# guomc9/CudaRayTracing

Hardware: AMD Instinct MI355X
Metric: Mrays/sec (higher is better)
Workload: dtype f32

## Files before the change

cudaraytracing_amd/csrc/crt_internal.h:

```cpp
#ifndef CRT_INTERNAL_H
#define CRT_INTERNAL_H
#include <cstdlib>
#include "crt_mega3.h"

#include <cstddef>
#include <string>
#include <vector>

extern "C" void crt_set_last_error_(const char* msg);

namespace crtk {

struct HipFail {
    hipError_t e;
    const char* what;
};
#define HIP_CHECK(call)                                          \
    do {                                                         \
        hipError_t e_ = (call);                                  \
        if (e_ != hipSuccess) throw HipFail{e_, #call};          \
    } while (0)

inline int fail(int status, const std::string& msg)
{
    crt_set_last_error_(msg.c_str());
    return status;
}
inline int fail_hip(const HipFail& f) { return fail(CRT_ERR_HIP, std::string(f.what) + ": " + hipGetErrorString(f.e)); }
template <class Body> int hip_guard(Body body)
{
    try { return body(); } catch (const HipFail& f) { return fail_hip(f); }
}

template <typename T> struct DevBuf {
    T* p = nullptr;
    size_t n = 0;
    void alloc(size_t count)
    {
        release();
        if (count == 0) count = 1;
        HIP_CHECK(hipMalloc((void**)&p, count * sizeof(T)));
        n = count;
        debug_fill();
    }
    void debug_fill()
    {
        static const char* e = std::getenv("CRT_DEBUG_FILL");
        if (!e || !*e) return;
        if (e[0] == 's') { HIP_CHECK(hipDeviceSynchronize()); return; }
        if (e[0] == 'u' && !uncached) return;
        if (e[0] == 'c' && uncached) return;
        const char* v = (e[0] == 'u' || e[0] == 'c') ? e + 1 : e;
        HIP_CHECK(hipMemset(p, std::atoi(v) & 0xff, n * sizeof(T)));
    }
    void ensure(size_t count)
    {
        if (n < count) alloc(count);
    }
    void ensure_uncached(size_t count)
    {
        if (n >= count && uncached) return;
        release();
        if (count == 0) count = 1;
        HIP_CHECK(hipExtMallocWithFlags((void**)&p, count * sizeof(T), hipDeviceMallocUncached));
        n = count;
        uncached = true;
        debug_fill();
    }
    bool uncached = false;
    template <typename Row> T* upload(const std::vector<Row>& v)
    {
        static_assert(sizeof(Row) == sizeof(T) && alignof(T) % alignof(Row) == 0, "upload is a byte copy");
        alloc(v.size());
        if (!v.empty()) HIP_CHECK(hipMemcpy(p, v.data(), v.size() * sizeof(T), hipMemcpyHostToDevice));
        return p;
    }
    T* upload(const T* h, size_t count)
    {
        if (!h) return nullptr;
        alloc(count);
        HIP_CHECK(hipMemcpy(p, h, count * sizeof(T), hipMemcpyHostToDevice));
        return p;
    }
    void download(T* h, size_t count) const
    {
        if (h) HIP_CHECK(hipMemcpy(h, p, count * sizeof(T), hipMemcpyDeviceToHost));
    }
    void release()
    {
        if (p) { (void)hipFree(p); p = nullptr; n = 0; uncached = false; }
    }
    ~DevBuf() { release(); }
};

const int kMaxBatch = 64;

}

#include "crt_stages.h"

namespace crtk {

#define REFILL_MIN 32
#define LEAF_MIN 24
#define SLOT_SHARDS 64
#define SLOT_STRIDE 32
// ... 84 lines not shown
```

cudaraytracing_amd/csrc/crt_mega3.h:

```cpp
#ifndef CRT_MEGA3_H
#define CRT_MEGA3_H
#include "crt_path.h"
#include "crt_item_order.h"

namespace crtk {

struct MParams {
    LParams P;
    DevScene sc;
    unsigned long long* counters;
    int2* spill;
    uint32_t spill_stride;
    int32_t stack_cap;
    int32_t logic_min, leaf_min;
};

#define POOL_LV 4

#define PH3_INNER 0
#define PH3_LEAF 1
#define PH3_LA 2
#define PH3_LB 3
#define PH3_LC 4
#define PH3_N 5
// ... 32 lines not shown
    int node[POOL3_P];
    stk_t stk[LV][POOL3_P];
    uint32_t D[POOL3_P];
    uint8_t ring[PH3_N + 1][POOL3_QCAP];
    uint32_t waitq;
    __device__ __forceinline__ uint8_t* rq(const int p) { return ring[p]; }
};
typedef Pool3LdsT<false> Pool3Lds;
static_assert(sizeof(Pool3LdsT<true>) == sizeof(Pool3Lds), "16-bit stack entries: twice the levels in the same bytes");
static_assert(sizeof(Pool3Lds) * 4 * CRT_WAVES <= 160 * 1024, "the pool does not fit CRT_WAVES waves per SIMD into 160 KiB of LDS");

#ifndef LEAFQ_CAP
#define LEAFQ_CAP 256
#endif
static_assert((LEAFQ_CAP & (LEAFQ_CAP - 1)) == 0 && LEAFQ_CAP >= 128, "leaf queue: a power of two, room for half a batch of inner steps");
constexpr int LEAFQ_FIRST = 48;
static_assert(LEAFQ_FIRST >= 1 && LEAFQ_FIRST + 64 + 4 <= LEAFQ_CAP, "leaf queue: LEAFQ_FIRST - 1 entries + a reference-arithmetic batch + one lane's four entries must fit LEAFQ_CAP");
constexpr int VISIT2_MIN = 44;
constexpr int CHAIN_MIN = 44;
#define RD_PEND_SHIFT 8
#define RD_PEND_MASK 0x3ff00u
#define RD_FIN 0x8000000u
#define LEAF_REC_MAX 0x7fffffu
template <bool R16_, bool RING_>
struct Pool4LdsT {
    static constexpr bool R16 = R16_;
    static constexpr bool DEC = true;
    static constexpr int P = RING_ ? 148 : 152;
    static constexpr int QCAP = (P + 3) & ~3;
    static constexpr int LV = R16_ ? 6 : 3;
    typedef typename std::conditional<R16_, short, int>::type stk_t;
    float4 A[P];
    float4 B[P];
    unsigned long long best[P];
    stk_t stk[LV][P];
    uint32_t D[P];
    uint32_t leafq[LEAFQ_CAP + 1];
    uint8_t ring[(RING_ ? 5 : 4)][QCAP];
    uint32_t waitq;
    __device__ __forceinline__ uint8_t* rq(const int p) { return ring[p == PH3_INNER ? 0 : p - 1]; }
};
static_assert(sizeof(Pool4LdsT<true, false>) * 4 * CRT_WAVES <= 160 * 1024 && sizeof(Pool4LdsT<true, true>) * 4 * CRT_WAVES <= 160 * 1024 &&
              sizeof(Pool4LdsT<false, false>) * 4 * CRT_WAVES <= 160 * 1024 && sizeof(Pool4LdsT<false, true>) * 4 * CRT_WAVES <= 160 * 1024,
              "the DEC pool does not fit CRT_WAVES waves per SIMD into 160 KiB of LDS");
static_assert(Pool4LdsT<true, false>::P <= 256, "ray ids of a pool must fit a byte");

struct MParams3 {
    MParams M;
    int* spill;
    uint32_t force_exact;
    int32_t dbg_loads, dbg_valu;
};

static_assert(offsetof(MParams3, dbg_loads) == 756 && offsetof(MParams3, dbg_valu) == 760, "tools/bbprof/instrument.py reads the counter buffer's address from these two kernel-argument dwords");


typedef void (*Mega3Kernel)(const MParams3);
struct Mega3Variant {
    uint32_t key;
    Mega3Kernel kern;
    uint32_t pool_p;
    int lds_levels;
};
const Mega3Variant* mega3_variant(int mode, bool stats, bool all, bool query, bool r16, bool ring = false, bool dec = false, bool impl = false);
bool bbprof_launch(Mega3Kernel kern, MParams3 M3, uint32_t blocks, hipStream_t st);
void launch_order_items(bool ring, uint32_t blocks, hipStream_t st, const LParams& P, const OrderClasses& C, uint32_t* list, unsigned int* cnt);

}
#endif
```

cudaraytracing_amd/csrc/crt_mega3_logic.h:

```cpp
#ifndef CRT_MEGA3_LOGIC_H
#define CRT_MEGA3_LOGIC_H
#include "crt_mega3_math.h"
#include "crt_mega3_wave.h"

namespace crtk {

struct NewRay {
    F3 o, d;
    float tl;
    uint32_t kind, flags;
};


template <bool QUERY = false>
__device__ __forceinline__ uint32_t route_done(uint32_t rec_flags)
{
    if (QUERY) return PH3_LC;
    return ((rec_flags >> RR_ROUTE_SHIFT) & 3u) + (uint32_t)PH3_LA;
}
__device__ __forceinline__ uint32_t route_bits(uint32_t nr_flags)
{
    const uint32_t r = (nr_flags & RF_SHADOW) ? ((nr_flags & RF_LAST) ? 1u : 0u) : ((nr_flags & RF_PROBE) ? 0u : 2u);
    return r << RR_ROUTE_SHIFT;
}
// ... 15 lines not shown
    const int ref = (MODE != 1 && finite && !force_exact) ? (IMPL ? sc.root4i : sc.root4) : sc.root3_exact;
    bool answered = false;
    float T = FLT_MAX;
    if (MODE != 1 && nr.kind == RAY_SHADOW) {
        flags |= RF_ANYHIT;
        T = nr.tl;
        answered = !(nr.tl == nr.tl) || nr.tl == -pinf() || (nr.flags & RF_SKIP) != 0;
    }
    if constexpr (LDS::DEC) {
        static_assert(!LDS::DEC || MODE == 2, "decoupled leaves: CRT_TRAVERSAL_EXACT");
        if (ref < 0) flags |= RF_EXACT;
        S.A[id] = make_float4(nr.o.x, nr.o.y, nr.o.z, (flags & RF_ANYHIT) ? T : pinf());
        S.B[id] = make_float4(nr.d.x, nr.d.y, nr.d.z, __int_as_float(ref));
        S.best[id] = (unsigned long long)0x7f7fffffu << 32;
        S.D[id] = flags;
        enters_exact = false;
        if (answered) return route_done<QUERY>(flags);
        enters_exact = (flags & RF_EXACT) != 0;
        return PH3_INNER;
    } else {
    S.A[id] = make_float4(nr.o.x, nr.o.y, nr.o.z, T);
    S.B[id] = make_float4(nr.d.x, nr.d.y, nr.d.z, __int_as_float(-1));
    S.node[id] = ref;
    S.D[id] = flags;
    enters_exact = false;
    if (answered) return route_done<QUERY>(flags);
    enters_exact = MODE != 1 && (flags & RF_EXACT) != 0;
    return ref >= 0 ? PH3_INNER : PH3_LEAF;
    }
}

template <class LDS>
__device__ __forceinline__ void ray_result(LDS& S, const uint32_t id, float4& qa, float4& qb)
{
    qa = S.A[id]; qb = S.B[id];
    if constexpr (LDS::DEC) {
        const unsigned long long b = S.best[id];
        qa.w = __uint_as_float((uint32_t)(b >> 32));
        qb.w = __uint_as_float(~(uint32_t)b);
    }
}
template <bool QUERY>
__device__ __forceinline__ uint32_t route_complete(const uint32_t rec_flags, const bool has_hit)
{
    if (QUERY) return PH3_LC;
    const uint32_t r = (rec_flags >> RR_ROUTE_SHIFT) & 3u;
    return (has_hit ? (r & 1u) : r) + (uint32_t)PH3_LA;
}


#define ST_TL_INF (1u << 12)

__device__ __forceinline__ F3 finish_path_m3(const LParams& P, const Tables<false>& tb, const uint32_t slot, const int deepest, const bool emissive, const F3 ke,
                                            const bool have_ld, const F3 ld)
{
    const Pool& pl = P.pool;
    if (deepest < 0) return f3(0.0f, 0.0f, 0.0f);
    F3 L;
    if (emissive) L = seed_emitter(deepest, ke);
    else if (have_ld) L = seed_direct(ld);
    else {
        const float4 a = gld_rec(&pl.rec_a[(size_t)deepest * pl.n + slot]);
        L = seed_direct(f3(a.x, a.y, a.z));
    }
    for (int v = deepest - 1; v >= 0; v -= CRT_FINISH_PF) {
        float4 a[CRT_FINISH_PF], fm[CRT_FINISH_PF];
        float cs[CRT_FINISH_PF];
#pragma unroll
        for (int j = 0; j < CRT_FINISH_PF; j++) {
            const int vj = v - j > 0 ? v - j : 0;
            a[j] = gld_rec(&pl.rec_a[(size_t)vj * pl.n + slot]);
            cs[j] = gld(&pl.rec_c[(size_t)vj * pl.n + slot]);
        }
#pragma unroll
        for (int j = 0; j < CRT_FINISH_PF; j++) fm[j] = mat_row(tb, TNM_MAT(__float_as_uint(a[j].w)), 0);
#pragma unroll
        for (int j = 0; j < CRT_FINISH_PF; j++) {
            if (v - j >= 0) L = indirect_step(L, f3(fm[j].x, fm[j].y, fm[j].z), cs[j], P.p_rr, f3(a[j].x, a[j].y, a[j].z));
        }
    }
    return L;
}


template <int MODE, bool RING = false>
__device__ __forceinline__ uint32_t logic_A(const LParams& P, const Tables<false>& tb, const uint32_t g, const float4 qa, const float4 qb, NewRay& nr,
                                            PathCounters& cnt, const bool trace_all)
{
    const DevScene& sc = P.sc;
    const Pool& pl = P.pool;
    constexpr bool TRI_CC = MODE != 1;
    const float4 la = gld(&pl.la[g]);
    const uint4 idv = load_path_id<RING, !TRI_CC>(P, g);
    const float4 cc = gld(&pl.cc[g]);
    const uint32_t st = __float_as_uint(la.w);
    const uint32_t stage = (st >> 8) & 15u;
    const uint32_t vtri_old = TRI_CC ? ((st & 0xfffu) == ((uint32_t)ST_HIT << 8) ? 0u : __float_as_uint(cc.w)) : idv.w;
    const float4 vn = gld(&sc.tri_nm[vtri_old]);
    const float res_t = qa.w;
    const int res_tri = __float_as_int(qb.w);
    const float4 gq_hit = gld(&sc.tri_nm[res_tri >= 0 ? res_tri : 0]);
    const uint32_t mat_old = min(TNM_MAT(__float_as_uint(vn.w)), P.n_mats - 1u);
    const uint32_t mat_cur = stage == ST_HIT ? TNM_MAT(__float_as_uint(gq_hit.w)) : mat_old;
    uint32_t tnm_cur = stage == ST_HIT ? __float_as_uint(gq_hit.w) : __float_as_uint(vn.w);
    float4 m0_cur = mat_row(tb, mat_cur, 0);
    const uint32_t n_nee = (uint32_t)(sc.n_lights * P.lsn);
    const uint32_t q_next = stage == ST_SHADOW ? (st >> 16) + 1 : 0u;
    uint4 lg_next = make_uint4(0u, 1u, 0u, 0u);
    if (n_nee > 0) {
        if (sc.n_lights == 1) {
            const crt_u4v_ l0_ = *(const __attribute__((address_space(4))) crt_u4v_*)tb.lights;
            lg_next = make_uint4(l0_.x, l0_.y, l0_.z, l0_.w);
        } else lg_next = gld(&tb.lights[fast_div(q_next < n_nee ? q_next : 0u, P.lsn_div.m, P.lsn_div.sh)]);
    }
    Lane s;
    s.depth = st & 255u; s.q = st >> 16; s.stage = stage;
    s.Ld = f3(la.x, la.y, la.z);
    s.nrm = f3(vn.x, vn.y, vn.z); s.mat = TNM_MAT(__float_as_uint(vn.w));
    s.pixel_index = idv.x; s.k = idv.y; s.item = idv.z;
    s.ro = f3(qa.x, qa.y, qa.z); s.tl = 0.0f;
    s.rd = f3(qb.x, qb.y, qb.z);
    s.pos = s.ro; s.vtri = vtri_old; s.c = f3(0.0f, 0.0f, 0.0f); s.kind = RAY_NONE;
    bool do_enter = false;
    if (stage == ST_SHADOW) {
        const bool blocked = TRI_CC ? shadow_blocked_bit((st & ST_TL_INF) != 0u, res_tri) : shadow_blocked<MODE>(cc.w, res_t, res_tri);
        if (!blocked) s.Ld = add3(s.Ld, f3(cc.x, cc.y, cc.z));
        s.q++;
    } else if (stage == ST_HIT) {
        const F3 pos = add3(s.ro, scalel3(res_t, s.rd));
        do_enter = true;
        if (s.depth > 0) {
            const size_t pr = (size_t)(s.depth - 1) * pl.n + g;
            const F3 pn = s.nrm;
            const float cos_prev = cos_to_next(s.ro, pos, pn);
            gst_rec(&pl.rec_c[pr], cos_prev);
            if (TNM_SPECULAR(__float_as_uint(vn.w))) {
                const float ns = mat_row(tb, s.mat, 0).w;
                const float4 pb = gld_rec(&pl.rec_b[pr]);
                const F3 refd = probe_dir(P.seed, s.pixel_index, s.k, s.depth - 1, ns, f3(pb.x, pb.y, pb.z), pn);
                gst_rec(&pl.rec_b[(size_t)s.depth * pl.n + g], make_float4(s.rd.x, s.rd.y, s.rd.z, 0.0f));
                gst(&pl.vx[g], make_float4(pos.x, pos.y, pos.z, __int_as_float(res_tri)));
                gst(&pl.la[g], make_float4(s.Ld.x, s.Ld.y, s.Ld.z, __uint_as_float(s.depth | ((uint32_t)ST_PROBE << 8) | (s.q << 16))));
                nr.o = s.ro; nr.d = unit3(refd);  nr.tl = 0.0f; nr.kind = RAY_CLOSEST; nr.flags = RF_PROBE;
                return PH3_NONE;
            }
        }
        s.pos = pos; s.vtri = (uint32_t)res_tri;
    } else {
        const float4 vx = gld(&pl.vx[g]);
        s.pos = f3(vx.x, vx.y, vx.z); s.vtri = __float_as_uint(vx.w);
        if (res_tri >= 0) {
            const int hmat = gld(&sc.tri_mat[res_tri]);
            const float4 h1 = mat_row(tb, hmat, 1);
            if (__float_as_uint(h1.w) & 1u) {
                const float4 h2 = mat_row(tb, hmat, 2);
                const size_t pr = (size_t)(s.depth - 1) * pl.n + g;
                const F3 pn = s.nrm;
                const float4 pm0 = mat_row(tb, s.mat, 0), pm1 = mat_row(tb, s.mat, 1);
                const F3 temp = probe_term(pn, f3(pm1.x, pm1.y, pm1.z), f3(h2.x, h2.y, h2.z), s.ro, s.rd, res_t, pm0.w);
                float4 a = gld_rec(&pl.rec_a[pr]);
                a.x = a.x + temp.x; a.y = a.y + temp.y; a.z = a.z + temp.z;
                gst_rec(&pl.rec_a[pr], a);
            }
        }
        const float4 pb = gld_rec(&pl.rec_b[(size_t)s.depth * pl.n + g]);
        s.rd = f3(pb.x, pb.y, pb.z);
        do_enter = true;
    }
    if (do_enter) {
        float4 gq = gq_hit;
        if (stage == ST_PROBE) {
            gq = gld(&sc.tri_nm[s.vtri]);
            m0_cur = mat_row(tb, TNM_MAT(__float_as_uint(gq.w)), 0); tnm_cur = __float_as_uint(gq.w);
        }
        s.nrm = f3(gq.x, gq.y, gq.z);
        s.mat = TNM_MAT(__float_as_uint(gq.w));
        if (TNM_SPECULAR(tnm_cur)) gst_rec(&pl.rec_b[(size_t)s.depth * pl.n + g], make_float4(s.rd.x, s.rd.y, s.rd.z, 0.0f));
        if (!TRI_CC) store_path_tri(P, g, s.vtri);
        if (TNM_EMITTER(tnm_cur)) {
            gst(&pl.la[g], make_float4(TRI_CC ? __uint_as_float(s.vtri) : 0.0f, 0.0f, 0.0f, __uint_as_float(s.depth | ((uint32_t)ST_FIN << 8) | (1u << 16))));
            return PH3_LC;
        }
        s.Ld = f3(0.0f, 0.0f, 0.0f);
        s.q = 0;
        if (n_nee == 0) {
            gst(&pl.la[g], make_float4(0.0f, 0.0f, 0.0f, __uint_as_float(s.depth | ((uint32_t)ST_NEED << 8))));
            if (TRI_CC) gst(&pl.cc[g].w, __uint_as_float(s.vtri));
            nr.o = s.pos;
            return PH3_LB;
        }
    }
    constexpr int LA_LOOP_MIN = 16;
    const float4 m0 = m0_cur;
    bool skip;
    for (bool first = true;; first = false) {
        if (first) setup_shadow_lg(P, s, f3(m0.x, m0.y, m0.z), lg_next);
        else setup_shadow(P, tb, s, f3(m0.x, m0.y, m0.z));
        skip = MODE != 1 && !trace_all && (s.c.x == 0.0f && s.c.y == 0.0f && s.c.z == 0.0f);
        if (!skip) break;
        cnt.untraced++;
        if (__popcll(__builtin_amdgcn_ballot_w64(true)) < LA_LOOP_MIN) break;
        cnt.rays++; cnt.shadow++;
        s.q++;
        if (s.q == n_nee) {
            gst(&pl.la[g], make_float4(s.Ld.x, s.Ld.y, s.Ld.z, __uint_as_float(s.depth | ((uint32_t)ST_NEED << 8))));
            if (TRI_CC) gst(&pl.cc[g].w, __uint_as_float(s.vtri));
            nr.o = s.pos;
            return PH3_LB;
        }
    }
    gst(&pl.la[g], make_float4(s.Ld.x, s.Ld.y, s.Ld.z, __uint_as_float(s.depth | ((uint32_t)ST_SHADOW << 8) | (s.q << 16) | ((TRI_CC && s.tl == pinf()) ? ST_TL_INF : 0u))));
    gst(&pl.cc[g], make_float4(s.c.x, s.c.y, s.c.z, TRI_CC ? __uint_as_float(s.vtri) : s.tl));
    nr.o = s.ro; nr.d = s.rd; nr.tl = s.tl; nr.kind = RAY_SHADOW;
    nr.flags = RF_SHADOW | (s.q + 1 == n_nee ? RF_LAST : 0u) | (skip ? RF_SKIP : 0u);
    return PH3_NONE;
}

template <int MODE, bool RING = false>
__device__ __forceinline__ uint32_t logic_B(const LParams& P, const uint32_t g, const float4 qa, const float4 qb, NewRay& nr)
{
    const Pool& pl = P.pool;
    constexpr bool TRI_CC = MODE != 1;
    const float4 la = gld(&pl.la[g]);
    const uint4 idv = load_path_id<RING, !TRI_CC>(P, g);
    const float4 cc = gld(&pl.cc[g]);
    const uint32_t st = __float_as_uint(la.w);
    const uint32_t stage = (st >> 8) & 15u;
    uint32_t depth = st & 255u;
    F3 Ld = f3(la.x, la.y, la.z);
    if (stage == ST_SHADOW) {
        const bool blocked = TRI_CC ? shadow_blocked_bit((st & ST_TL_INF) != 0u, __float_as_int(qb.w)) : shadow_blocked<MODE>(cc.w, qa.w, __float_as_int(qb.w));
        if (!blocked) Ld = add3(Ld, f3(cc.x, cc.y, cc.z));
    }
    U4 rb;
    if (roulette(P.seed, idv.x, idv.y, depth, P.p_rr, rb)) {
        gst(&pl.la[g], make_float4(Ld.x, Ld.y, Ld.z, __uint_as_float(depth | ((uint32_t)ST_FIN << 8))));
        return PH3_LC;
    }
    const float4 vn = gld(&P.sc.tri_nm[TRI_CC ? __float_as_uint(cc.w) : idv.w]);
    const float4 vx = qa;
    gst_rec(&pl.rec_a[(size_t)depth * pl.n + g], make_float4(Ld.x, Ld.y, Ld.z, vn.w));
    const F3 ndir = bounce_dir(f3(vn.x, vn.y, vn.z), rb);
    depth++;
    gst(&pl.la[g], make_float4(Ld.x, Ld.y, Ld.z, __uint_as_float(depth | ((uint32_t)ST_HIT << 8))));
    nr.o = f3(vx.x, vx.y, vx.z); nr.d = unit3(ndir);  nr.tl = 0.0f; nr.kind = RAY_CLOSEST; nr.flags = 0;
    return PH3_NONE;
}

enum { LC_DEAD = 0, LC_RAY = 1, LC_WAIT = 2 };
template <int MODE, bool RING>
__device__ __forceinline__ int logic_C(const LParams& P, const Tables<false>& tb, const uint32_t g, PathCounters& cnt, NewRay& nr, uint32_t& fin_key)
{
    constexpr bool TRI_CC = MODE != 1;
    const Pool& pl = P.pool;
    const float4 la = gld(&pl.la[g]);
    const uint4 idv = load_path_id<RING, !TRI_CC>(P, g);
    const uint32_t st = __float_as_uint(la.w);
    const uint32_t stage = (st >> 8) & 15u;
    const uint32_t depth = st & 255u;
    constexpr bool ring = RING;
    const bool waiting = ring && stage == ST_WAIT;
    const uint32_t home_ = RING ? blockIdx.x & (P.ring_shards - 1u) : blockIdx.x & (ITEM_SHARDS - 1);
    const uint32_t lo_ = home_ * P.items_per_shard, hi_ = min(lo_ + P.items_per_shard, P.n_items);
    const unsigned long long gmask_ = __ballot(!waiting);
    const int lane_ = threadIdx.x & 63;
    const uint32_t grank_ = (uint32_t)__popcll(gmask_ & ((1ull << lane_) - 1ull));
    unsigned int pre_base_ = 0;
    const bool pre_ok_ = lo_ < P.n_items && gmask_ != 0ull;
    if (pre_ok_ && lane_ == __ffsll((long long)gmask_) - 1) pre_base_ = __hip_atomic_fetch_add((CRT_GAS unsigned int*)(P.item_next + home_ * ITEM_STRIDE), (unsigned int)__popcll(gmask_), __ATOMIC_RELAXED, __HIP_MEMORY_SCOPE_AGENT);
    uint32_t home_word_ = 0;
    if (RING) home_word_ = ring_load(P.ring_state + home_ * ITEM_STRIDE);
    if (stage != ST_NEW && !waiting) {
        int deepest = (int)depth;
        bool emissive = false;
        F3 ke = f3(0.0f, 0.0f, 0.0f);
        if (stage == ST_HIT) deepest = (int)depth - 1;
        else if ((st >> 16) & 1u) {
            emissive = true;
            const float4 m2 = mat_row(tb, TNM_MAT(__float_as_uint(gld(&P.sc.tri_nm[TRI_CC ? __float_as_uint(la.x) : idv.w]).w)), 2);
            ke = f3(m2.x, m2.y, m2.z);
        }
        const F3 L = finish_path_m3(P, tb, g, deepest, emissive, ke, stage == ST_FIN && !emissive, f3(la.x, la.y, la.z));
        if (ring) {
            const uint32_t sh = fast_div(idv.z, P.items_per_shard_div.m, P.items_per_shard_div.sh), c = idv.z - sh * P.items_per_shard;
            const uint32_t s = fast_div(c, P.spsh_div.m, P.spsh_div.sh), rs = s & P.ring_mask;
            Rad3* Lr = P.L + (size_t)rs * P.ring_stride + (size_t)sh * P.spsh + (c - s * P.spsh);
            ring_store12(Lr, L.x, L.y, L.z);
            fin_key = (sh << 16) | rs;
        } else {
            store_radiance(&P.L[idv.z], L.x, L.y, L.z);
        }
    }
    bool first_ = pre_ok_ && !waiting;
    for (;;) {
        uint32_t item = ITEM_NONE;
        if (waiting) item = idv.z;
        else {
            if (first_) {
                const unsigned long long idx_ = (unsigned long long)lo_ + (unsigned int)__builtin_amdgcn_readfirstlane((int)pre_base_) + grank_;
                if (idx_ < hi_) item = (uint32_t)idx_;
                first_ = false;
            }
            if (item == ITEM_NONE) item = RING ? grab_item_ring(P.item_next, P.items_per_shard, P.ring_shards, home_)
                                               : grab_item(P.item_next, P.items_per_shard, P.n_items, blockIdx.x & (ITEM_SHARDS - 1));
            if (item == ITEM_NONE) return LC_DEAD;
            if (P.item_list) {
                const uint32_t sh_ = fast_div(item, P.items_per_shard_div.m, P.items_per_shard_div.sh);
                const uint32_t slo_ = sh_ * P.items_per_shard, shi_ = min(slo_ + P.items_per_shard, P.n_items);
                const uint32_t wlo_ = shi_ - min(P.order_window, shi_ - slo_);
                if (item >= wlo_) item = __hip_atomic_load((CRT_GAS const unsigned int*)&P.item_list[sh_ * P.order_window + (item - wlo_)], __ATOMIC_RELAXED, __HIP_MEMORY_SCOPE_AGENT);
            }
        }
        bool valid; uint32_t pi, pj, pixel_index, k;
        decode_item<RING>(P, item, pixel_index, k, valid, pi, pj);
        if (!valid) continue;
        if (ring && !ring_gate_open(P, item, home_, home_word_)) {
            if (!waiting) {
                store_path_id<!TRI_CC>(P, g, item);
                gst(&pl.la[g], make_float4(0.0f, 0.0f, 0.0f, __uint_as_float((uint32_t)ST_WAIT << 8)));
            }
            return LC_WAIT;
        }
        cnt.paths++;
        if (!waiting) store_path_id<!TRI_CC>(P, g, item);
        const F3 wd = camera_dir(P, pixel_index, k, pi, pj);
        gst(&pl.la[g], make_float4(0.0f, 0.0f, 0.0f, __uint_as_float((uint32_t)ST_HIT << 8)));
        nr.o = f3(P.eye[0], P.eye[1], P.eye[2]); nr.d = unit3(wd);  nr.tl = 0.0f; nr.kind = RAY_CLOSEST; nr.flags = 0;
        return LC_RAY;
    }
}

__device__ __forceinline__ bool query_C(const LParams& P, const uint32_t g, const float4 qa, const float4 qb, NewRay& nr)
{
    const Pool& pl = P.pool;
    const float4 la = gld(&pl.la[g]);
// ... 14 lines not shown
```

cudaraytracing_amd/csrc/crt_path.h:

```cpp
#ifndef CRT_PATH_H
#define CRT_PATH_H
#include "../../include/crt.h"
#include "crt_accel.h"
#include "crt_device.h"
#include "crt_trace.h"

#include <hip/hip_runtime.h>

#include <cfloat>
#include <cstddef>
#include <cstdint>
#include <type_traits>

namespace crtk {
using namespace crtdev;

enum { C_RAYS = 0, C_SHADOW, C_PROBE, C_INNER, C_LEAF, C_TESTS, C_HITS, C_PATHS, C_ALIVE, C_MAXSP, C_SUMSP, C_CYC_LOGIC, C_CYC_LEAF, C_CYC_INNER, C_CYC_OTHER,
       C_DIAG , C_UNTRACED = C_DIAG + 20, C_COUNT };
#define CNT_SHARDS 256
#define CNT_STRIDE 40
#define ITEM_SHARDS 64
#define ITEM_STRIDE 32

enum { ST_DEAD = 0, ST_NEW = 1, ST_HIT = 2, ST_PROBE = 3, ST_SHADOW = 4, ST_FIN = 5, ST_NEED = 6, ST_WAIT = 7, ST_COUNT_ };
static_assert(ST_COUNT_ <= 16, "a stage is kept in 4 bits");
enum { RAY_NONE = 0, RAY_CLOSEST = 1, RAY_SHADOW = 2 };
#define ITEM_NONE 0xffffffffu

struct Pool {
    float4* ro;
    float4* rd;
    float4* vx;
    float4* la;
    float4* cc;
    float4* vn;
    uint4* id;
    float2* res;
    float4* rec_a;
    float4* rec_b;
    float* rec_c;
    uint32_t n;
};

struct Rad3 {
    float x, y, z;
};
static_assert(sizeof(Rad3) == 12 && alignof(Rad3) == 4, "a radiance entry is three floats");

struct LParams {
    DevScene sc;
    Pool pool;
    float eye[3];
    float inv_view[9];
    float scale, ar;
    uint32_t width, height;
    float p_rr;
    int32_t lsn;
    float inv_lsn_pow2;
    uint32_t pad_;
    uint64_t seed;
    uint32_t rank, world, tiles_x, n_tiles;
    uint32_t nslots;
    uint32_t sample_begin;
    uint32_t n_items;
    uint32_t items_per_shard;
    uint32_t n_mats;
    FastDiv lsn_div, nslots_div, tiles_x_div;
    unsigned int* item_next;
    union {
        Rad3* L;
        float4* L4;
    };
    unsigned long long* counters;
    const float4* q_o;
    const float4* q_d;
    const uint32_t* item_list;
    uint32_t order_window;
    FastDiv items_per_shard_div;
    uint32_t ring_mask;
    uint32_t spsh;
    FastDiv spsh_div;
    uint32_t ring_shards;
    uint32_t ring_stride;
    uint32_t n_samples;
    uint32_t tail_first;
    float spp_f;
    uint32_t ring_pad_;
    unsigned int* ring_done;
    unsigned int* ring_state;
    float* accum;
};

struct TParams {
    DevScene sc;
    Pool pool;
// ... 446 lines not shown
```

cudaraytracing_amd/csrc/crt_render.hip:

```cpp
#include "crt_render.h"

#include <algorithm>
#include <cfloat>
#include <cstdio>
#include <cstdlib>
#include <cstring>
#include <string>
#include <vector>

using namespace crtdev;
using namespace crtk;
using namespace crtlayout;

static bool use_ref16(const crt_scene* sc, int mode, bool dec = false)
{
    if (mode == 1 || !sc->can(dec ? CAP_REF16_INNER : CAP_REF16)) return false;
    const char* e = std::getenv("CRT_REF16");
    const char* f = std::getenv("CRT_REF32");
    if (f && f[0] == '1') return false;
    return dec || !(e && e[0] == '0');
}

namespace {

// ... 271 lines not shown
    const uint32_t forced = env_u32("CRT_COMMIT_RING_LOG2", 0);
    if (forced) rs = 1u << std::min(16u, forced);
    const uint64_t per_shard = (uint64_t)spsh * s_count;
    const bool fits32 = per_shard * shards < 0xffffffffull;
    if ((forced || (prm->flags & CRT_FLAG_BOUNDED_RADIANCE)) && rs < s_count && fits32) { ring.samples = rs; ring.spsh = spsh; ring.shards = shards; }
    return ring;
}

constexpr uint32_t kOrderWindow = 1u << 19;
OrderClasses order_classes_from_env()
{
    OrderClasses C;
    std::memset(&C, 0, sizeof(C));
    const uint32_t dflt[] = {1, 2, 3, 5, 9};
    C.n = (uint32_t)(sizeof(dflt) / sizeof(dflt[0]));
    for (uint32_t c = 0; c < C.n; c++) C.lo[c] = dflt[c];
    const char* e = std::getenv("CRT_ORDER_CLASSES");
    if (!e || !*e) return C;
    OrderClasses E;
    std::memset(&E, 0, sizeof(E));
    E.n = 1; E.lo[0] = 1;
    for (const char* p = e; *p;) {
        char* end = nullptr;
        const long v = std::strtol(p, &end, 10);
        if (end == p || E.n == ORDER_CLASSES_MAX || v <= (long)E.lo[E.n - 1] || v > CRT_BOUNCE_STACK_SIZE) return C;
        E.lo[E.n++] = (uint32_t)v;
        p = end;
        if (*p == ',') p++;
        else if (*p) return C;
    }
    return E.n >= 2 ? E : C;
}

void render_mega(Frame& f)
{
    crt_scene* sc = f.sc;
    const crt_params* prm = f.prm;
    const Shard& sh = f.sh;
    const RingPlan& ring = f.ring;
    hipStream_t st = f.st;
    const bool timing = f.stats != nullptr;
    auto chunk_items = [&](uint32_t k, uint32_t ns) { return f.src ? f.src->items(k, ns) : (uint32_t)((uint64_t)ns * sh.nslots); };
    uint64_t most_items = ring.samples ? (uint64_t)(f.s_end - f.s_begin) * sh.nslots : f.cap;
    if (f.src) {
        most_items = 0;
        for (uint32_t s0 = f.s_begin, k = 0; s0 < f.s_end; s0 += f.chunk, k++) most_items = std::max<uint64_t>(most_items, chunk_items(k, std::min(f.chunk, f.s_end - s0)));
    }
    const MegaPlan mp = plan_mega3(sc, prm->traversal, f.want_stats, (prm->flags & CRT_FLAG_TRACE_ALL) != 0, false, ring.samples != 0, most_items, env_u32("CRT_MEGA_BLOCKS_PER_CU", 64));
    const uint32_t lanes = mp.lanes;
    sc->p_vx.ensure(lanes); sc->p_la.ensure(lanes); sc->p_cc.ensure(lanes); sc->p_id.ensure(lanes);
    sc->p_rec_a.ensure((size_t)lanes * CRT_BOUNCE_STACK_SIZE);
    sc->p_rec_b.ensure((size_t)lanes * CRT_BOUNCE_STACK_SIZE);
    sc->p_rec_c.ensure((size_t)lanes * CRT_BOUNCE_STACK_SIZE);
    sc->spill[0].ensure(mp.spill_entries);
    LParams P = frame_lparams(f);
    P.pool.vx = sc->p_vx.p; P.pool.la = sc->p_la.p; P.pool.cc = sc->p_cc.p; P.pool.vn = sc->p_vn.p; P.pool.id = sc->p_id.p;
    P.pool.rec_a = sc->p_rec_a.p; P.pool.rec_b = sc->p_rec_b.p; P.pool.rec_c = sc->p_rec_c.p; P.pool.n = lanes;
    MParams M;
    std::memset(&M, 0, sizeof(M));
    M.sc = sc->dev; M.counters = sc->counters.p; M.spill = sc->spill[0].p; M.spill_stride = lanes; M.stack_cap = mp.lds_levels;
    hipEvent_t e0 = nullptr, e3 = nullptr;
    if (timing) {
        ensure_chunk_events(sc, (f.s_end - f.s_begin + f.chunk - 1) / f.chunk);
        e0 = sc->ev[0]; e3 = sc->ev[3];
        HIP_CHECK(hipEventRecord(e0, st));
    }
    uint32_t launches = 0;
    for (uint32_t s0 = f.s_begin; s0 < f.s_end; s0 += f.chunk) {
        uint32_t ns = std::min(f.chunk, f.s_end - s0);
        set_chunk(P, s0, chunk_items(launches, ns));
        if (ring.samples) {
            P.items_per_shard = ring.spsh * ns;
            P.n_items = P.items_per_shard * ring.shards;
            P.ring_mask = ring.samples - 1u; P.spsh = ring.spsh; P.spsh_div = make_fastdiv(ring.spsh); P.ring_shards = ring.shards;
            P.ring_stride = ring.spsh * ring.shards; P.n_samples = ns; P.tail_first = P.items_per_shard; P.spp_f = (float)prm->spp;
            sc->ring_done.ensure_uncached((size_t)ring.shards * ring.samples);
            sc->ring_state.ensure_uncached((size_t)ring.shards * ITEM_STRIDE);
            P.ring_done = sc->ring_done.p; P.ring_state = sc->ring_state.p; P.accum = sc->accum.p; P.L = sc->ring_L.p;
            std::vector<unsigned int>& state = sc->ring_state_host;
            state.assign((size_t)ring.shards * ITEM_STRIDE, 0u);
            for (uint32_t lt = 0; lt < sh.local_tiles; lt++) state[(size_t)(lt * 64u / ring.spsh) * ITEM_STRIDE + 1] += tile_pixels(f.A, lt);
            HIP_CHECK(hipMemcpyAsync(sc->ring_state.p, state.data(), state.size() * sizeof(unsigned int), hipMemcpyHostToDevice, st));
            HIP_CHECK(hipMemsetAsync(sc->ring_done.p, 0, (size_t)ring.shards * ring.samples * sizeof(unsigned int), st));
        }
        P.item_list = nullptr;
        sc->order_classes = 0; sc->order_window = 0;
        if (f.src) {
            P.order_window = P.items_per_shard;
            sc->order_key.valid = 0;
            sc->item_list.ensure(P.n_items);
            f.src->fill(sc->item_list.p, s0, ns, P.n_items, st);
            HIP_CHECK(hipGetLastError());
            P.item_list = sc->item_list.p;
        } else {
            const char* eo = std::getenv("CRT_ITEM_ORDER");
            const bool order = !(eo && eo[0] == '0');
            if (order && P.n_items > 0) {
                P.order_window = std::min<uint32_t>(P.items_per_shard, env_u32("CRT_ORDER_WINDOW", kOrderWindow));
                if (ring.samples) {
                    P.order_window = std::min<uint32_t>(P.order_window, (ring.samples / 2u) * ring.spsh);
                    P.tail_first = P.items_per_shard - P.order_window;
                }
                P.items_per_shard_div = make_fastdiv(std::max(1u, P.items_per_shard));
                const uint32_t n_sh = ring.samples ? ring.shards : (uint32_t)ITEM_SHARDS;
                const OrderClasses C = order_classes_from_env();
                ItemOrderKey key;
                std::memset(&key, 0, sizeof(key));
                key.valid = 1; key.seed = P.seed; key.stream = (uint64_t)(uintptr_t)st; key.sample_begin = P.sample_begin; key.n_items = P.n_items;
                key.items_per_shard = P.items_per_shard; key.order_window = P.order_window; key.shards = n_sh; key.ring = ring.samples ? 1u : 0u;
                key.spsh = ring.samples ? ring.spsh : 0u; key.nslots = P.nslots; key.rank = P.rank; key.world = P.world; key.tiles_x = P.tiles_x;
// ... 31 lines not shown
            M3.force_exact = (prm->flags & CRT_FLAG_FORCE_EXACT) ? 1u : 0u;
            M3.dbg_loads = 0; M3.dbg_valu = 0;
            if (!bbprof_launch(mp.kern, M3, mp.blocks, st)) hipLaunchKernelGGL(mp.kern, dim3(mp.blocks), dim3(64), 0, st, M3);
        }
        HIP_CHECK(hipGetLastError());
        if (s0 + ns >= f.s_end) HIP_CHECK(hipEventRecord(sc->ev_k1, st));
        if (timing) HIP_CHECK(hipEventRecord(sc->ev_chunk[2 * launches + 1], st));
        launches++;
        sc->last_launches = launches;
        accumulate_chunk(f, s0, ns);
    }
    if (f.stats) {
        HIP_CHECK(hipEventRecord(e3, st));
        HIP_CHECK(hipMemcpyAsync(sc->h_counters, sc->counters.p, kCountersBytes, hipMemcpyDeviceToHost, st));
        HIP_CHECK(hipStreamSynchronize(st));
        double kernel_ms = 0.0;
        for (uint32_t c = 0; c < launches; c++) {
            float ms = 0.0f;
            HIP_CHECK(hipEventElapsedTime(&ms, sc->ev_chunk[2 * c], sc->ev_chunk[2 * c + 1]));
            kernel_ms += ms;
        }
        float total = 0.0f;
        HIP_CHECK(hipEventElapsedTime(&total, e0, e3));
        read_stats(sc, f.stats, true, kernel_ms, 0.0, total, launches);
    }
}

void render_wavefront(Frame& f)
{
    crt_scene* sc = f.sc;
    const crt_params* prm = f.prm;
    const Shard& sh = f.sh;
    hipStream_t st = f.st;
    const bool timing = f.stats != nullptr;
    const uint32_t pool_log2 = std::min(26u, std::max(8u, env_u32("CRT_POOL_LOG2", 22)));
    const uint32_t pool_n = (uint32_t)std::min<uint64_t>((f.cap + 255) / 256 * 256, 1ull << pool_log2);
    const int batch_max = (int)std::min<uint32_t>(kMaxBatch, env_u32("CRT_ROUND_BATCH", 16));
    int batch = batch_max;
    unsigned long long alive_seen = 0;
    const int n_halves = (pool_n >= 2 * 65536u && env_u32("CRT_STREAMS", 2) >= 2) ? 2 : 1;
    const uint32_t half_n = n_halves == 2 ? ((pool_n / 2 + 255) / 256 * 256) : pool_n;
    const size_t slots = (size_t)half_n * n_halves;
    sc->p_ro.ensure(slots); sc->p_rd.ensure(slots); sc->p_vx.ensure(slots); sc->p_la.ensure(slots); sc->p_cc.ensure(slots); sc->p_res.ensure(slots);
    sc->p_vn.ensure(slots); sc->p_id.ensure(slots);
    sc->p_rec_a.ensure(slots * CRT_BOUNCE_STACK_SIZE);
    sc->p_rec_b.ensure(slots * CRT_BOUNCE_STACK_SIZE);
    Pool pools[2];
    for (int h = 0; h < n_halves; h++) {
        Pool& pool = pools[h];
        const size_t o = (size_t)h * half_n;
        pool.ro = sc->p_ro.p + o; pool.rd = sc->p_rd.p + o; pool.vx = sc->p_vx.p + o; pool.la = sc->p_la.p + o; pool.cc = sc->p_cc.p + o;
        pool.vn = sc->p_vn.p + o; pool.id = sc->p_id.p + o; pool.res = sc->p_res.p + o;
        pool.rec_a = sc->p_rec_a.p + o * CRT_BOUNCE_STACK_SIZE; pool.rec_b = sc->p_rec_b.p + o * CRT_BOUNCE_STACK_SIZE;
        pool.n = half_n;
    }
    hipStream_t streams[2] = {st, sc->aux_stream};
    LParams P = frame_lparams(f);
    const bool lds_tables = sc->n_mats <= LOGIC_TABLE_MAX && (uint32_t)sc->dev.n_lights <= LOGIC_TABLE_MAX;
    TraceSetup TS[2];
    LParams PH[2];
    for (int h = 0; h < n_halves; h++) TS[h] = make_trace_setup(sc, pools[h], prm->traversal, f.want_stats, h, n_halves);

    double trace_ms = 0.0, logic_ms = 0.0;
    uint32_t trace_launches = 0;
    hipEvent_t ev_begin = nullptr, ev_end = nullptr;
    if (timing) {
        ev_begin = sc->ev[4 * kMaxBatch + 2];
        ev_end = sc->ev[4 * kMaxBatch + 3];
        HIP_CHECK(hipEventRecord(ev_begin, st));
    }
    const dim3 pool_grid((half_n + 255) / 256);
    const int evs_per_half = 2 * kMaxBatch + 1;
    for (uint32_t s0 = f.s_begin; s0 < f.s_end; s0 += f.chunk) {
        uint32_t ns = std::min(f.chunk, f.s_end - s0);
        set_chunk(P, s0, (uint32_t)((uint64_t)ns * P.nslots));
        HIP_CHECK(hipMemsetAsync(sc->item_next.p, 0, (size_t)ITEM_SHARDS * ITEM_STRIDE * sizeof(unsigned int), st));
        for (int h = 0; h < n_halves; h++) {
            PH[h] = P;
            PH[h].pool = pools[h];
            launch_pool_init(pool_grid.x, st, pools[h]);
        }
        HIP_CHECK(hipGetLastError());
        for (;;) {
            if (n_halves == 2) {
                HIP_CHECK(hipEventRecord(sc->ev_fork, st));
                HIP_CHECK(hipStreamWaitEvent(sc->aux_stream, sc->ev_fork, 0));
            }
            for (int h = 0; h < n_halves; h++)
                if (timing) HIP_CHECK(hipEventRecord(sc->ev[h * evs_per_half], streams[h]));
            for (int b = 0; b < batch; b++) {
                for (int h = 0; h < n_halves; h++) {
                    hipStream_t hs = streams[h];
                    hipEvent_t* ev = sc->ev.data() + h * evs_per_half;
                    launch_logic(lds_tables, pool_grid.x, hs, PH[h]);
                    if (timing) HIP_CHECK(hipEventRecord(ev[2 * b + 1], hs));
                    launch_trace_pass(sc, TS[h], hs);
                    if (timing) HIP_CHECK(hipEventRecord(ev[2 * b + 2], hs));
                }
            }
            HIP_CHECK(hipGetLastError());
            if (n_halves == 2) {
                HIP_CHECK(hipEventRecord(sc->ev_join, sc->aux_stream));
                HIP_CHECK(hipStreamWaitEvent(st, sc->ev_join, 0));
            }
            HIP_CHECK(hipMemcpyAsync(sc->h_counters, sc->counters.p, kCountersBytes, hipMemcpyDeviceToHost, st));
            HIP_CHECK(hipStreamSynchronize(st));
// ... 404 lines not shown
```

cudaraytracing_amd/csrc/crt_scene.h:

```cpp
#ifndef CRT_SCENE_H
#define CRT_SCENE_H
#include "crt_internal.h"
#include "crt_scene_layout.h"

#include <cstdlib>
#include <vector>

struct FrameMark {
    uint32_t samples = 0, spp = 0, width = 0, height = 0, rank = 0, world = 1, tiled = 0;
    bool valid = false;
    void set(const crt_params* prm, uint32_t samples_, bool tiled_)
    {
        samples = samples_; spp = prm->spp; width = prm->width; height = prm->height;
        rank = prm->rank; world = prm->world; tiled = tiled_ ? 1u : 0u;
    }
    std::string in_flight(const std::string& tail) const
    {
        return samples == 0 ? std::string("no frame is in flight on the handle")
                            : "the frame in flight holds samples [0, " + std::to_string(samples) + ") of spp " + std::to_string(spp) + tail;
    }
};

struct ItemOrderKey {
    uint64_t seed, stream;
    uint32_t valid, sample_begin, n_items, items_per_shard, order_window, shards, ring, spsh, nslots, rank, world, tiles_x, n_tiles, width, height, p_rr_bits;
    uint32_t n_classes, class_lo[8];
    uint32_t pad_;
};

struct ItemResults {
    crtk::DevBuf<float> words;
    crtk::Rad3* radiance(size_t n) { words.ensure(n * 3); return reinterpret_cast<crtk::Rad3*>(words.p); }
    float4* answers(size_t n) { words.ensure(n * 4); return reinterpret_cast<float4*>(words.p); }
};

const size_t kAovAccRows = 3, kAovAccRowsShading = 4;

struct crt_scene {
    int device = 0;
    crtk::DevBuf<float4> nodes, tri_geo, mats, ltri, nodes3, leaf_geo, tri_nm, nodes4, nodes4i, leaf_geo_i;
    crtk::DevBuf<int32_t> rec_map;
    uint32_t max_leaf = 0;
    crtk::DevBuf<int32_t> tri_mat, leaf_count;
    crtk::DevBuf<uint4> lights;
    crtk::DevBuf<float4> p_ro, p_rd, p_vx, p_la, p_cc, p_vn, p_rec_a, p_rec_b;
    crtk::DevBuf<float> p_rec_c;
    ItemResults L;
    crtk::DevBuf<uint4> p_id;
    uint32_t n_mats = 0;
    crtk::DevBuf<float2> p_res;
    crtk::DevBuf<float> accum;
    crtk::DevBuf<float4> aov_acc;
    crtk::DevBuf<float4> aovs_state;
    crtk::DevBuf<int2> aovs_aux;
    crtk::DevBuf<uint32_t> aovs_item;
    crtk::DevBuf<unsigned int> aovs_count;
    unsigned int* h_aovs_count = nullptr;
    crtk::DevBuf<unsigned long long> counters;
    crtk::DevBuf<unsigned int> item_next;
    crtk::DevBuf<uint32_t> item_list;
    crtk::DevBuf<unsigned int> ring_done, ring_state;
    crtk::DevBuf<crtk::Rad3> ring_L;
    std::vector<unsigned int> ring_state_host;
    uint64_t last_radiance_bytes = 0;
    uint32_t last_ring_samples = 0;
    crtk::DevBuf<unsigned int> order_cnt;
    ItemOrderKey order_key{};
    uint64_t order_built = 0, order_reused = 0;
    uint32_t order_classes = 0, order_window = 0;
    crtk::DevBuf<unsigned int> slot_next[2];
    crtk::DevBuf<int2> spill[2];
    hipStream_t aux_stream = nullptr;
    hipEvent_t ev_fork = nullptr, ev_join = nullptr;
    hipEvent_t ev_k0 = nullptr, ev_k1 = nullptr;
    uint32_t last_launches = 0;
    int n_cus = 0;
    unsigned long long* h_counters = nullptr;
    crtdev::DevScene dev{};
    crt_tree_scalars scalars{};
    int stack_cap = 0;
    uint32_t n_tris = 0;
    crt_accel_info accel{};
    bool can(uint32_t cap) const { return (accel.layout_caps & cap) != 0; }
    FrameMark acc;
    crtk::DevBuf<float> accum_q;
    FrameMark var;
    crtk::DevBuf<float> accum_h;
    FrameMark half;
    crtk::DevBuf<uint32_t> ad_nsamp, ad_list;
    crtk::DevBuf<unsigned int> ad_count;
    unsigned int* h_ad_count = nullptr;
    crtk::DevBuf<unsigned int> map_hist, map_cursor;
    unsigned int* h_map = nullptr;
    size_t h_map_words = 0;
    std::vector<hipEvent_t> ev;
    std::vector<hipEvent_t> ev_chunk;
    ~crt_scene()
    {
        for (hipEvent_t e : ev) (void)hipEventDestroy(e);
// ... 75 lines not shown
```

Baseline: 13590.

## Pack per-slot shallow vertex records into one cache line and defer rec_a store

Adds a RecLine struct that holds each slot's first six path-vertex rec_a and rec_c records in a single 128-byte line, with rec_a_at/rec_c_at routing shallow depths to it. The rec_a store moves from the hit stage to the next bounce, where it is written together with rec_c, and finish_path no longer reloads rec_a for the deepest vertex. The goal is fewer scattered strided memory transactions during path finishing and bounce bookkeeping. The cost is an extra per-slot buffer, plus a debug-fill sync and a change to kernel-argument offsets.

```diff
diff --git a/cudaraytracing_amd/csrc/crt_internal.h b/cudaraytracing_amd/csrc/crt_internal.h
--- a/cudaraytracing_amd/csrc/crt_internal.h
+++ b/cudaraytracing_amd/csrc/crt_internal.h
@@ -52,6 +52,7 @@
         if (e[0] == 'c' && uncached) return;
         const char* v = (e[0] == 'u' || e[0] == 'c') ? e + 1 : e;
         HIP_CHECK(hipMemset(p, std::atoi(v) & 0xff, n * sizeof(T)));
+        HIP_CHECK(hipDeviceSynchronize());
     }
     void ensure(size_t count)
     {
diff --git a/cudaraytracing_amd/csrc/crt_mega3.h b/cudaraytracing_amd/csrc/crt_mega3.h
--- a/cudaraytracing_amd/csrc/crt_mega3.h
+++ b/cudaraytracing_amd/csrc/crt_mega3.h
@@ -108,7 +108,7 @@
     int32_t dbg_loads, dbg_valu;
 };
 
-static_assert(offsetof(MParams3, dbg_loads) == 756 && offsetof(MParams3, dbg_valu) == 760, "tools/bbprof/instrument.py reads the counter buffer's address from these two kernel-argument dwords");
+static_assert(offsetof(MParams3, dbg_loads) == 764 && offsetof(MParams3, dbg_valu) == 768, "tools/bbprof/instrument.py reads the counter buffer's address from these two kernel-argument dwords");
 
 
 typedef void (*Mega3Kernel)(const MParams3);
diff --git a/cudaraytracing_amd/csrc/crt_mega3_logic.h b/cudaraytracing_amd/csrc/crt_mega3_logic.h
--- a/cudaraytracing_amd/csrc/crt_mega3_logic.h
+++ b/cudaraytracing_amd/csrc/crt_mega3_logic.h
@@ -91,25 +91,19 @@
 #define ST_TL_INF (1u << 12)
 
 __device__ __forceinline__ F3 finish_path_m3(const LParams& P, const Tables<false>& tb, const uint32_t slot, const int deepest, const bool emissive, const F3 ke,
-                                            const bool have_ld, const F3 ld)
+                                            const F3 ld)
 {
     const Pool& pl = P.pool;
     if (deepest < 0) return f3(0.0f, 0.0f, 0.0f);
-    F3 L;
-    if (emissive) L = seed_emitter(deepest, ke);
-    else if (have_ld) L = seed_direct(ld);
-    else {
-        const float4 a = gld_rec(&pl.rec_a[(size_t)deepest * pl.n + slot]);
-        L = seed_direct(f3(a.x, a.y, a.z));
-    }
+    F3 L = emissive ? seed_emitter(deepest, ke) : seed_direct(ld);
     for (int v = deepest - 1; v >= 0; v -= CRT_FINISH_PF) {
         float4 a[CRT_FINISH_PF], fm[CRT_FINISH_PF];
         float cs[CRT_FINISH_PF];
 #pragma unroll
         for (int j = 0; j < CRT_FINISH_PF; j++) {
             const int vj = v - j > 0 ? v - j : 0;
-            a[j] = gld_rec(&pl.rec_a[(size_t)vj * pl.n + slot]);
-            cs[j] = gld(&pl.rec_c[(size_t)vj * pl.n + slot]);
+            a[j] = gld_rec(rec_a_at(pl, (uint32_t)vj, slot));
+            cs[j] = gld(rec_c_at(pl, (uint32_t)vj, slot));
         }
 #pragma unroll
         for (int j = 0; j < CRT_FINISH_PF; j++) fm[j] = mat_row(tb, TNM_MAT(__float_as_uint(a[j].w)), 0);
@@ -172,7 +166,8 @@
             const size_t pr = (size_t)(s.depth - 1) * pl.n + g;
             const F3 pn = s.nrm;
             const float cos_prev = cos_to_next(s.ro, pos, pn);
-            gst_rec(&pl.rec_c[pr], cos_prev);
+            gst_rec(rec_a_at(pl, s.depth - 1, g), make_float4(la.x, la.y, la.z, vn.w));
+            gst_rec(rec_c_at(pl, s.depth - 1, g), cos_prev);
             if (TNM_SPECULAR(__float_as_uint(vn.w))) {
                 const float ns = mat_row(tb, s.mat, 0).w;
                 const float4 pb = gld_rec(&pl.rec_b[pr]);
@@ -193,13 +188,13 @@
             const float4 h1 = mat_row(tb, hmat, 1);
             if (__float_as_uint(h1.w) & 1u) {
                 const float4 h2 = mat_row(tb, hmat, 2);
-                const size_t pr = (size_t)(s.depth - 1) * pl.n + g;
                 const F3 pn = s.nrm;
                 const float4 pm0 = mat_row(tb, s.mat, 0), pm1 = mat_row(tb, s.mat, 1);
                 const F3 temp = probe_term(pn, f3(pm1.x, pm1.y, pm1.z), f3(h2.x, h2.y, h2.z), s.ro, s.rd, res_t, pm0.w);
-                float4 a = gld_rec(&pl.rec_a[pr]);
+                float4* const ra = rec_a_at(pl, s.depth - 1, g);
+                float4 a = gld_rec(ra);
                 a.x = a.x + temp.x; a.y = a.y + temp.y; a.z = a.z + temp.z;
-                gst_rec(&pl.rec_a[pr], a);
+                gst_rec(ra, a);
             }
         }
         const float4 pb = gld_rec(&pl.rec_b[(size_t)s.depth * pl.n + g]);
@@ -278,7 +273,6 @@
     }
     const float4 vn = gld(&P.sc.tri_nm[TRI_CC ? __float_as_uint(cc.w) : idv.w]);
     const float4 vx = qa;
-    gst_rec(&pl.rec_a[(size_t)depth * pl.n + g], make_float4(Ld.x, Ld.y, Ld.z, vn.w));
     const F3 ndir = bounce_dir(f3(vn.x, vn.y, vn.z), rb);
     depth++;
     gst(&pl.la[g], make_float4(Ld.x, Ld.y, Ld.z, __uint_as_float(depth | ((uint32_t)ST_HIT << 8))));
@@ -319,7 +313,7 @@
             const float4 m2 = mat_row(tb, TNM_MAT(__float_as_uint(gld(&P.sc.tri_nm[TRI_CC ? __float_as_uint(la.x) : idv.w]).w)), 2);
             ke = f3(m2.x, m2.y, m2.z);
         }
-        const F3 L = finish_path_m3(P, tb, g, deepest, emissive, ke, stage == ST_FIN && !emissive, f3(la.x, la.y, la.z));
+        const F3 L = finish_path_m3(P, tb, g, deepest, emissive, ke, f3(la.x, la.y, la.z));
         if (ring) {
             const uint32_t sh = fast_div(idv.z, P.items_per_shard_div.m, P.items_per_shard_div.sh), c = idv.z - sh * P.items_per_shard;
             const uint32_t s = fast_div(c, P.spsh_div.m, P.spsh_div.sh), rs = s & P.ring_mask;
diff --git a/cudaraytracing_amd/csrc/crt_path.h b/cudaraytracing_amd/csrc/crt_path.h
--- a/cudaraytracing_amd/csrc/crt_path.h
+++ b/cudaraytracing_amd/csrc/crt_path.h
@@ -26,6 +26,14 @@
 static_assert(ST_COUNT_ <= 16, "a stage is kept in 4 bits");
 enum { RAY_NONE = 0, RAY_CLOSEST = 1, RAY_SHADOW = 2 };
 #define ITEM_NONE 0xffffffffu
+
+#define CRT_REC_LINE_DEPTH 6
+struct alignas(128) RecLine {
+    float4 a[CRT_REC_LINE_DEPTH];
+    float c[CRT_REC_LINE_DEPTH];
+    float spare[2];
+};
+static_assert(sizeof(RecLine) == 128 && alignof(RecLine) == 128, "a slot's vertex records are one cache line");
 
 struct Pool {
     float4* ro;
@@ -39,8 +47,17 @@
     float4* rec_a;
     float4* rec_b;
     float* rec_c;
+    RecLine* rec_v;
     uint32_t n;
 };
+__device__ __forceinline__ float4* rec_a_at(const Pool& pl, const uint32_t depth, const uint32_t slot)
+{
+    return depth < (uint32_t)CRT_REC_LINE_DEPTH ? &pl.rec_v[slot].a[depth] : &pl.rec_a[(size_t)depth * pl.n + slot];
+}
+__device__ __forceinline__ float* rec_c_at(const Pool& pl, const uint32_t depth, const uint32_t slot)
+{
+    return depth < (uint32_t)CRT_REC_LINE_DEPTH ? &pl.rec_v[slot].c[depth] : &pl.rec_c[(size_t)depth * pl.n + slot];
+}
 
 struct Rad3 {
     float x, y, z;
diff --git a/cudaraytracing_amd/csrc/crt_render.hip b/cudaraytracing_amd/csrc/crt_render.hip
--- a/cudaraytracing_amd/csrc/crt_render.hip
+++ b/cudaraytracing_amd/csrc/crt_render.hip
@@ -347,10 +347,11 @@
     sc->p_rec_a.ensure((size_t)lanes * CRT_BOUNCE_STACK_SIZE);
     sc->p_rec_b.ensure((size_t)lanes * CRT_BOUNCE_STACK_SIZE);
     sc->p_rec_c.ensure((size_t)lanes * CRT_BOUNCE_STACK_SIZE);
+    sc->p_rec_v.ensure(lanes);
     sc->spill[0].ensure(mp.spill_entries);
     LParams P = frame_lparams(f);
     P.pool.vx = sc->p_vx.p; P.pool.la = sc->p_la.p; P.pool.cc = sc->p_cc.p; P.pool.vn = sc->p_vn.p; P.pool.id = sc->p_id.p;
-    P.pool.rec_a = sc->p_rec_a.p; P.pool.rec_b = sc->p_rec_b.p; P.pool.rec_c = sc->p_rec_c.p; P.pool.n = lanes;
+    P.pool.rec_a = sc->p_rec_a.p; P.pool.rec_b = sc->p_rec_b.p; P.pool.rec_c = sc->p_rec_c.p; P.pool.rec_v = sc->p_rec_v.p; P.pool.n = lanes;
     MParams M;
     std::memset(&M, 0, sizeof(M));
     M.sc = sc->dev; M.counters = sc->counters.p; M.spill = sc->spill[0].p; M.spill_stride = lanes; M.stack_cap = mp.lds_levels;
@@ -488,6 +489,7 @@
         pool.ro = sc->p_ro.p + o; pool.rd = sc->p_rd.p + o; pool.vx = sc->p_vx.p + o; pool.la = sc->p_la.p + o; pool.cc = sc->p_cc.p + o;
         pool.vn = sc->p_vn.p + o; pool.id = sc->p_id.p + o; pool.res = sc->p_res.p + o;
         pool.rec_a = sc->p_rec_a.p + o * CRT_BOUNCE_STACK_SIZE; pool.rec_b = sc->p_rec_b.p + o * CRT_BOUNCE_STACK_SIZE;
+        pool.rec_c = nullptr; pool.rec_v = nullptr;
         pool.n = half_n;
     }
     hipStream_t streams[2] = {st, sc->aux_stream};
diff --git a/cudaraytracing_amd/csrc/crt_scene.h b/cudaraytracing_amd/csrc/crt_scene.h
--- a/cudaraytracing_amd/csrc/crt_scene.h
+++ b/cudaraytracing_amd/csrc/crt_scene.h
@@ -45,6 +45,7 @@
     crtk::DevBuf<uint4> lights;
     crtk::DevBuf<float4> p_ro, p_rd, p_vx, p_la, p_cc, p_vn, p_rec_a, p_rec_b;
     crtk::DevBuf<float> p_rec_c;
+    crtk::DevBuf<crtk::RecLine> p_rec_v;
     ItemResults L;
     crtk::DevBuf<uint4> p_id;
     uint32_t n_mats = 0;
```

New measurement: 13600 (median of 3 runs). About the same (+0.0%).
